# thunlp/OpenMatch

Measured on NVIDIA H100. Metric: queries/sec top-1000 over 8.8M x 768 corpus, higher is better.
Workload: dtype f16

## Files before the change

openmatch_b200/csrc/ptx.cuh:

```cuda
#pragma once
#include <cuda_runtime.h>
#include <cuda_bf16.h>
#include <stdint.h>

#ifndef OM_WAIT_TIMEOUT_CYCLES
#define OM_WAIT_TIMEOUT_CYCLES (1000000000ll)
#endif

namespace om {

static __device__ unsigned int om_dev_fault;

__device__ __forceinline__ uint32_t smem_u32(const void* p) {
  return static_cast<uint32_t>(__cvta_generic_to_shared(p));
}

__device__ __forceinline__ void mbar_init(uint64_t* bar, uint32_t count) {
  asm volatile("mbarrier.init.shared::cta.b64 [%0], %1;" ::"r"(smem_u32(bar)), "r"(count) : "memory");
}
__device__ __forceinline__ void fence_barrier_init() {
  asm volatile("fence.mbarrier_init.release.cluster;" ::: "memory");
}
__device__ __forceinline__ void fence_proxy_async_smem() {
  asm volatile("fence.proxy.async.shared::cta;" ::: "memory");
}
__device__ __forceinline__ void fence_proxy_async_global() {
  asm volatile("fence.proxy.async.global;" ::: "memory");
}
__device__ __forceinline__ void mbar_arrive_expect_tx(uint64_t* bar, uint32_t bytes) {
  asm volatile("mbarrier.arrive.expect_tx.shared::cta.b64 _, [%0], %1;" ::"r"(smem_u32(bar)), "r"(bytes)
               : "memory");
}
__device__ __forceinline__ void mbar_arrive(uint64_t* bar) {
  asm volatile("mbarrier.arrive.shared::cta.b64 _, [%0];" ::"r"(smem_u32(bar)) : "memory");
}
__device__ __forceinline__ bool mbar_try_wait(uint64_t* bar, uint32_t parity) {
  uint32_t done;
  asm volatile(
      "{\n\t"
      ".reg .pred P;\n\t"
      "mbarrier.try_wait.parity.shared::cta.b64 P, [%1], %2;\n\t"
      "selp.u32 %0, 1, 0, P;\n\t"
      "}\n"
      : "=r"(done)
      : "r"(smem_u32(bar)), "r"(parity)
      : "memory");
  return done != 0;
}
static __device__ __noinline__ void mbar_wait_slow(uint64_t* bar, uint32_t parity, uint32_t site) {
  const long long t0 = clock64();
  uint32_t spins = 0;
  while (!mbar_try_wait(bar, parity)) {
    if ((++spins & 1023u) != 0) continue;
    if (*reinterpret_cast<volatile unsigned int*>(&om_dev_fault) != 0u) return;
    if (clock64() - t0 > OM_WAIT_TIMEOUT_CYCLES) {
      atomicCAS(&om_dev_fault, 0u, (site << 16) | (blockIdx.x & 0xffffu) | 0x80000000u);
      return;
    }
  }
}
__device__ __forceinline__ void mbar_wait(uint64_t* bar, uint32_t parity, uint32_t site) {
  if (mbar_try_wait(bar, parity)) return;
  if (mbar_try_wait(bar, parity)) return;
  mbar_wait_slow(bar, parity, site);
}
__device__ __forceinline__ void mbar_wait_warp(uint64_t* bar, uint32_t parity, uint32_t site) {
  if ((threadIdx.x & 31u) == 0) {
    if (!mbar_try_wait(bar, parity)) {
      const long long t0 = clock64();
      uint32_t spins = 0;
      while (!mbar_try_wait(bar, parity)) {
        __nanosleep(64);
        if ((++spins & 1023u) != 0) continue;
        if (*reinterpret_cast<volatile unsigned int*>(&om_dev_fault) != 0u) break;
        if (clock64() - t0 > OM_WAIT_TIMEOUT_CYCLES) {
          atomicCAS(&om_dev_fault, 0u, (site << 16) | (blockIdx.x & 0xffffu) | 0x80000000u);
          break;
        }
      }
    }
  }
  __syncwarp();
}
static inline unsigned int read_clear_dev_fault() {
  unsigned int v = 0, z = 0;
  if (cudaMemcpyFromSymbol(&v, om_dev_fault, sizeof(v)) != cudaSuccess) return 0xffffffffu;
  if (v) cudaMemcpyToSymbol(om_dev_fault, &z, sizeof(z));
  return v;
}

__device__ __forceinline__ void tma_prefetch_desc(const void* tmap) {
  asm volatile("prefetch.tensormap [%0];" ::"l"(reinterpret_cast<uint64_t>(tmap)) : "memory");
}
__device__ __forceinline__ void tma_load_2d(void* smem_dst, const void* tmap, uint64_t* bar, int32_t c0,
                                            int32_t c1) {
  asm volatile(
      "cp.async.bulk.tensor.2d.shared::cluster.global.tile.mbarrier::complete_tx::bytes"
      " [%0], [%1, {%3, %4}], [%2];"
      ::"r"(smem_u32(smem_dst)), "l"(reinterpret_cast<uint64_t>(tmap)), "r"(smem_u32(bar)), "r"(c0), "r"(c1)
      : "memory");
}
__device__ __forceinline__ void tma_prefetch_l2_2d(const void* tmap, int32_t c0, int32_t c1) {
  asm volatile("cp.async.bulk.prefetch.tensor.2d.L2.global.tile [%0, {%1, %2}];" ::"l"(reinterpret_cast<uint64_t>(tmap)),
               "r"(c0), "r"(c1)
               : "memory");
}
__device__ __forceinline__ void tma_store_2d(const void* tmap, const void* smem_src, int32_t c0, int32_t c1) {
  asm volatile("cp.async.bulk.tensor.2d.global.shared::cta.tile.bulk_group [%0, {%2, %3}], [%1];" ::"l"(
                   reinterpret_cast<uint64_t>(tmap)),
               "r"(smem_u32(smem_src)), "r"(c0), "r"(c1)
               : "memory");
}
__device__ __forceinline__ void bulk_commit_group() { asm volatile("cp.async.bulk.commit_group;" ::: "memory"); }
__device__ __forceinline__ void bulk_wait_group_read0() { asm volatile("cp.async.bulk.wait_group.read 0;" ::: "memory"); }
__device__ __forceinline__ void bulk_wait_group0() { asm volatile("cp.async.bulk.wait_group 0;" ::: "memory"); }

__device__ __forceinline__ void tma_load_2d_multicast(void* smem_dst, const void* tmap, uint64_t* bar, int32_t c0,
                                                      int32_t c1, uint16_t cta_mask) {
  asm volatile(
      "cp.async.bulk.tensor.2d.shared::cluster.global.tile.mbarrier::complete_tx::bytes.multicast::cluster"
      " [%0], [%1, {%3, %4}], [%2], %5;"
      ::"r"(smem_u32(smem_dst)), "l"(reinterpret_cast<uint64_t>(tmap)), "r"(smem_u32(bar)), "r"(c0), "r"(c1),
      "h"(cta_mask)
      : "memory");
}

__device__ __forceinline__ uint32_t cluster_ctarank() {
  uint32_t r;
  asm volatile("mov.u32 %0, %%cluster_ctarank;" : "=r"(r));
  return r;
}
__device__ __forceinline__ uint32_t cluster_id_x() {
  uint32_t r;
  asm volatile("mov.u32 %0, %%clusterid.x;" : "=r"(r));
  return r;
}
__device__ __forceinline__ uint32_t cluster_count_x() {
  uint32_t r;
  asm volatile("mov.u32 %0, %%nclusterid.x;" : "=r"(r));
  return r;
}
__device__ __forceinline__ void cluster_sync_all() {
  asm volatile("barrier.cluster.arrive.release.aligned;\n\tbarrier.cluster.wait.acquire.aligned;" ::: "memory");
}
__device__ __forceinline__ void mbar_arrive_remote(uint64_t* bar, uint32_t rank) {
  asm volatile(
      "{\n\t.reg .b32 ra;\n\t"
      "mapa.shared::cluster.u32 ra, %0, %1;\n\t"
      "mbarrier.arrive.shared::cluster.b64 _, [ra];\n\t}\n"
      ::"r"(smem_u32(bar)), "r"(rank)
      : "memory");
}

__device__ __forceinline__ void wgmma_fence() { asm volatile("wgmma.fence.sync.aligned;" ::: "memory"); }
__device__ __forceinline__ void wgmma_commit() { asm volatile("wgmma.commit_group.sync.aligned;" ::: "memory"); }
template <int N>
__device__ __forceinline__ void wgmma_wait() {
  asm volatile("wgmma.wait_group.sync.aligned %0;" ::"n"(N) : "memory");
}
template <int R>
__device__ __forceinline__ void wgmma_fence_regs(float (&d)[R]) {
#pragma unroll
  for (int i = 0; i < R; ++i) asm volatile("" : "+f"(d[i])::"memory");
}

__host__ __device__ constexpr uint64_t wgmma_desc_base(uint32_t lbo_bytes, uint32_t sbo_bytes) {
  return (static_cast<uint64_t>((lbo_bytes >> 4) & 0x3fffu) << 16) |
         (static_cast<uint64_t>((sbo_bytes >> 4) & 0x3fffu) << 32) | (1ull << 62);
}
__device__ __forceinline__ uint64_t wgmma_desc(uint32_t smem_addr, uint64_t base) {
  return base | static_cast<uint64_t>((smem_addr & 0x3ffffu) >> 4);
}
constexpr uint64_t kDescKMajorSW128 = wgmma_desc_base(16, 1024);

template <int TA, int TB>
__device__ __forceinline__ void wgmma_m64n128k16_bf16(float (&d)[64], uint64_t a_desc, uint64_t b_desc, uint32_t accumulate) {
  asm volatile(
      "{\n\t.reg .pred p;\n\tsetp.ne.b32 p, %66, 0;\n\t"
      "wgmma.mma_async.sync.aligned.m64n128k16.f32.bf16.bf16 {%0, %1, %2, %3, %4, %5, %6, %7, %8, %9, %10, %11, %12, %13, %14, %15, %16, %17, %18, %19, %20, %21, %22, %23, %24, %25, %26, %27, %28, %29, %30, %31, %32, %33, %34, %35, %36, %37, %38, %39, %40, %41, %42, %43, %44, %45, %46, %47, %48, %49, %50, %51, %52, %53, %54, %55, %56, %57, %58, %59, %60, %61, %62, %63}, %64, %65, p, 1, 1, %67, %68;\n\t}\n"
      : "+f"(d[0]), "+f"(d[1]), "+f"(d[2]), "+f"(d[3]), "+f"(d[4]), "+f"(d[5]), "+f"(d[6]), "+f"(d[7]), "+f"(d[8]), "+f"(d[9]), "+f"(d[10]), "+f"(d[11]), "+f"(d[12]), "+f"(d[13]), "+f"(d[14]), "+f"(d[15]), "+f"(d[16]), "+f"(d[17]), "+f"(d[18]), "+f"(d[19]), "+f"(d[20]), "+f"(d[21]), "+f"(d[22]), "+f"(d[23]), "+f"(d[24]), "+f"(d[25]), "+f"(d[26]), "+f"(d[27]), "+f"(d[28]), "+f"(d[29]), "+f"(d[30]), "+f"(d[31]), "+f"(d[32]), "+f"(d[33]), "+f"(d[34]), "+f"(d[35]), "+f"(d[36]), "+f"(d[37]), "+f"(d[38]), "+f"(d[39]), "+f"(d[40]), "+f"(d[41]), "+f"(d[42]), "+f"(d[43]), "+f"(d[44]), "+f"(d[45]), "+f"(d[46]), "+f"(d[47]), "+f"(d[48]), "+f"(d[49]), "+f"(d[50]), "+f"(d[51]), "+f"(d[52]), "+f"(d[53]), "+f"(d[54]), "+f"(d[55]), "+f"(d[56]), "+f"(d[57]), "+f"(d[58]), "+f"(d[59]), "+f"(d[60]), "+f"(d[61]), "+f"(d[62]), "+f"(d[63])
      : "l"(a_desc), "l"(b_desc), "r"(accumulate), "n"(TA), "n"(TB));
}
template <int TA, int TB>
__device__ __forceinline__ void wgmma_m64n128k16_f16(float (&d)[64], uint64_t a_desc, uint64_t b_desc, uint32_t accumulate) {
  asm volatile(
      "{\n\t.reg .pred p;\n\tsetp.ne.b32 p, %66, 0;\n\t"
      "wgmma.mma_async.sync.aligned.m64n128k16.f32.f16.f16 {%0, %1, %2, %3, %4, %5, %6, %7, %8, %9, %10, %11, %12, %13, %14, %15, %16, %17, %18, %19, %20, %21, %22, %23, %24, %25, %26, %27, %28, %29, %30, %31, %32, %33, %34, %35, %36, %37, %38, %39, %40, %41, %42, %43, %44, %45, %46, %47, %48, %49, %50, %51, %52, %53, %54, %55, %56, %57, %58, %59, %60, %61, %62, %63}, %64, %65, p, 1, 1, %67, %68;\n\t}\n"
      : "+f"(d[0]), "+f"(d[1]), "+f"(d[2]), "+f"(d[3]), "+f"(d[4]), "+f"(d[5]), "+f"(d[6]), "+f"(d[7]), "+f"(d[8]), "+f"(d[9]), "+f"(d[10]), "+f"(d[11]), "+f"(d[12]), "+f"(d[13]), "+f"(d[14]), "+f"(d[15]), "+f"(d[16]), "+f"(d[17]), "+f"(d[18]), "+f"(d[19]), "+f"(d[20]), "+f"(d[21]), "+f"(d[22]), "+f"(d[23]), "+f"(d[24]), "+f"(d[25]), "+f"(d[26]), "+f"(d[27]), "+f"(d[28]), "+f"(d[29]), "+f"(d[30]), "+f"(d[31]), "+f"(d[32]), "+f"(d[33]), "+f"(d[34]), "+f"(d[35]), "+f"(d[36]), "+f"(d[37]), "+f"(d[38]), "+f"(d[39]), "+f"(d[40]), "+f"(d[41]), "+f"(d[42]), "+f"(d[43]), "+f"(d[44]), "+f"(d[45]), "+f"(d[46]), "+f"(d[47]), "+f"(d[48]), "+f"(d[49]), "+f"(d[50]), "+f"(d[51]), "+f"(d[52]), "+f"(d[53]), "+f"(d[54]), "+f"(d[55]), "+f"(d[56]), "+f"(d[57]), "+f"(d[58]), "+f"(d[59]), "+f"(d[60]), "+f"(d[61]), "+f"(d[62]), "+f"(d[63])
      : "l"(a_desc), "l"(b_desc), "r"(accumulate), "n"(TA), "n"(TB));
}
template <int TA, int TB>
__device__ __forceinline__ void wgmma_m64n256k16_f16(float (&d)[128], uint64_t a_desc, uint64_t b_desc, uint32_t accumulate) {
  asm volatile(
      "{\n\t.reg .pred p;\n\tsetp.ne.b32 p, %130, 0;\n\t"
      "wgmma.mma_async.sync.aligned.m64n256k16.f32.f16.f16 {%0, %1, %2, %3, %4, %5, %6, %7, %8, %9, %10, %11, %12, %13, %14, %15, %16, %17, %18, %19, %20, %21, %22, %23, %24, %25, %26, %27, %28, %29, %30, %31, %32, %33, %34, %35, %36, %37, %38, %39, %40, %41, %42, %43, %44, %45, %46, %47, %48, %49, %50, %51, %52, %53, %54, %55, %56, %57, %58, %59, %60, %61, %62, %63, %64, %65, %66, %67, %68, %69, %70, %71, %72, %73, %74, %75, %76, %77, %78, %79, %80, %81, %82, %83, %84, %85, %86, %87, %88, %89, %90, %91, %92, %93, %94, %95, %96, %97, %98, %99, %100, %101, %102, %103, %104, %105, %106, %107, %108, %109, %110, %111, %112, %113, %114, %115, %116, %117, %118, %119, %120, %121, %122, %123, %124, %125, %126, %127}, %128, %129, p, 1, 1, %131, %132;\n\t}\n"
      : "+f"(d[0]), "+f"(d[1]), "+f"(d[2]), "+f"(d[3]), "+f"(d[4]), "+f"(d[5]), "+f"(d[6]), "+f"(d[7]), "+f"(d[8]), "+f"(d[9]), "+f"(d[10]), "+f"(d[11]), "+f"(d[12]), "+f"(d[13]), "+f"(d[14]), "+f"(d[15]), "+f"(d[16]), "+f"(d[17]), "+f"(d[18]), "+f"(d[19]), "+f"(d[20]), "+f"(d[21]), "+f"(d[22]), "+f"(d[23]), "+f"(d[24]), "+f"(d[25]), "+f"(d[26]), "+f"(d[27]), "+f"(d[28]), "+f"(d[29]), "+f"(d[30]), "+f"(d[31]), "+f"(d[32]), "+f"(d[33]), "+f"(d[34]), "+f"(d[35]), "+f"(d[36]), "+f"(d[37]), "+f"(d[38]), "+f"(d[39]), "+f"(d[40]), "+f"(d[41]), "+f"(d[42]), "+f"(d[43]), "+f"(d[44]), "+f"(d[45]), "+f"(d[46]), "+f"(d[47]), "+f"(d[48]), "+f"(d[49]), "+f"(d[50]), "+f"(d[51]), "+f"(d[52]), "+f"(d[53]), "+f"(d[54]), "+f"(d[55]), "+f"(d[56]), "+f"(d[57]), "+f"(d[58]), "+f"(d[59]), "+f"(d[60]), "+f"(d[61]), "+f"(d[62]), "+f"(d[63]), "+f"(d[64]), "+f"(d[65]), "+f"(d[66]), "+f"(d[67]), "+f"(d[68]), "+f"(d[69]), "+f"(d[70]), "+f"(d[71]), "+f"(d[72]), "+f"(d[73]), "+f"(d[74]), "+f"(d[75]), "+f"(d[76]), "+f"(d[77]), "+f"(d[78]), "+f"(d[79]), "+f"(d[80]), "+f"(d[81]), "+f"(d[82]), "+f"(d[83]), "+f"(d[84]), "+f"(d[85]), "+f"(d[86]), "+f"(d[87]), "+f"(d[88]), "+f"(d[89]), "+f"(d[90]), "+f"(d[91]), "+f"(d[92]), "+f"(d[93]), "+f"(d[94]), "+f"(d[95]), "+f"(d[96]), "+f"(d[97]), "+f"(d[98]), "+f"(d[99]), "+f"(d[100]), "+f"(d[101]), "+f"(d[102]), "+f"(d[103]), "+f"(d[104]), "+f"(d[105]), "+f"(d[106]), "+f"(d[107]), "+f"(d[108]), "+f"(d[109]), "+f"(d[110]), "+f"(d[111]), "+f"(d[112]), "+f"(d[113]), "+f"(d[114]), "+f"(d[115]), "+f"(d[116]), "+f"(d[117]), "+f"(d[118]), "+f"(d[119]), "+f"(d[120]), "+f"(d[121]), "+f"(d[122]), "+f"(d[123]), "+f"(d[124]), "+f"(d[125]), "+f"(d[126]), "+f"(d[127])
      : "l"(a_desc), "l"(b_desc), "r"(accumulate), "n"(TA), "n"(TB));
}

template <int N>
__device__ __forceinline__ void setmaxnreg_dec() {
  asm volatile("setmaxnreg.dec.sync.aligned.u32 %0;" ::"n"(N));
}
template <int N>
__device__ __forceinline__ void setmaxnreg_inc() {
  asm volatile("setmaxnreg.inc.sync.aligned.u32 %0;" ::"n"(N));
}
__device__ __forceinline__ void wgmma_m64n64k16_bf16_rs(float (&d)[32], const uint32_t (&a)[4], uint64_t b_desc, uint32_t accumulate) {
  asm volatile(
      "{\n\t.reg .pred p;\n\tsetp.ne.b32 p, %37, 0;\n\t"
      "wgmma.mma_async.sync.aligned.m64n64k16.f32.bf16.bf16 {%0, %1, %2, %3, %4, %5, %6, %7, %8, %9, %10, %11, %12, %13, %14, %15, %16, %17, %18, %19, %20, %21, %22, %23, %24, %25, %26, %27, %28, %29, %30, %31}, {%32, %33, %34, %35}, %36, p, 1, 1, 0;\n\t}\n"
      : "+f"(d[0]), "+f"(d[1]), "+f"(d[2]), "+f"(d[3]), "+f"(d[4]), "+f"(d[5]), "+f"(d[6]), "+f"(d[7]), "+f"(d[8]), "+f"(d[9]), "+f"(d[10]), "+f"(d[11]), "+f"(d[12]), "+f"(d[13]), "+f"(d[14]), "+f"(d[15]), "+f"(d[16]), "+f"(d[17]), "+f"(d[18]), "+f"(d[19]), "+f"(d[20]), "+f"(d[21]), "+f"(d[22]), "+f"(d[23]), "+f"(d[24]), "+f"(d[25]), "+f"(d[26]), "+f"(d[27]), "+f"(d[28]), "+f"(d[29]), "+f"(d[30]), "+f"(d[31])
      : "r"(a[0]), "r"(a[1]), "r"(a[2]), "r"(a[3]), "l"(b_desc), "r"(accumulate));
}

__device__ __forceinline__ uint32_t pack_bf16x2(float lo, float hi) {
  __nv_bfloat162 v = __floats2bfloat162_rn(lo, hi);
  return *reinterpret_cast<uint32_t*>(&v);
}
__device__ __forceinline__ float2 fma2(float2 a, float2 b, float2 c) { return make_float2(fmaf(a.x, b.x, c.x), fmaf(a.y, b.y, c.y)); }
__device__ __forceinline__ float2 mul2(float2 a, float2 b) { return make_float2(__fmul_rn(a.x, b.x), __fmul_rn(a.y, b.y)); }
__device__ __forceinline__ float2 splat2(float x) { return make_float2(x, x); }

__device__ __forceinline__ void named_bar_sync(uint32_t id, uint32_t nthreads) {
  asm volatile("bar.sync %0, %1;" ::"r"(id), "r"(nthreads) : "memory");
}

}
```

openmatch_b200/csrc/scan_gemm.cuh:

```cuda
#pragma once
#include <cuda_fp16.h>

#include "scan_epilogue.cuh"

namespace om {

constexpr int kScanBlockN = 256;
constexpr int kScanStages = 3;
constexpr int kScanABytes = kBlockM * kBlockK * 2;
constexpr int kScanBBytes = kScanBlockN * kBlockK * 2;
constexpr int kScanStageBytes = kScanABytes + kScanBBytes;
constexpr int kScanConsumers = 256;
constexpr int kScanStash = 4;
constexpr int kScanStashOffset = kScanStages * kScanStageBytes;
constexpr int kScanStashBytes = 2 * 2 * kScanStash * kScanConsumers * 8;
constexpr int kScanBarOffset = kScanStashOffset + kScanStashBytes;
constexpr int kScanSmemBytes = kScanBarOffset + 2 * kScanStages * 8 + 1024;
static_assert(kScanSmemBytes <= 232448, "scan ring + stash exceed the 227 KB of shared memory an H100 block may use");

template <int H>
__device__ __forceinline__ float scan_pick(const float (&acc)[128], int i) {
  float a[32], b[16], c[8], d[4], e[2];
#pragma unroll
  for (int j = 0; j < 32; ++j) a[j] = (i & 1) ? acc[4 * j + 2 * H + 1] : acc[4 * j + 2 * H];
#pragma unroll
  for (int j = 0; j < 16; ++j) b[j] = (i & 2) ? a[2 * j + 1] : a[2 * j];
#pragma unroll
  for (int j = 0; j < 8; ++j) c[j] = (i & 4) ? b[2 * j + 1] : b[2 * j];
#pragma unroll
  for (int j = 0; j < 4; ++j) d[j] = (i & 8) ? c[2 * j + 1] : c[2 * j];
#pragma unroll
  for (int j = 0; j < 2; ++j) e[j] = (i & 16) ? d[2 * j + 1] : d[2 * j];
  return (i & 32) ? e[1] : e[0];
}

template <int H>
__device__ __forceinline__ int scan_filter_row(const float (&acc)[128], float t, int row, int lim, int q4, int col0,
                                               unsigned long long* stash, unsigned long long* cand, int* count,
                                               int* overflow, int C, uint32_t row_base) {
  float mx = acc[2 * H];
#pragma unroll
  for (int j = 0; j < 32; ++j) mx = fmaxf(mx, fmaxf(acc[4 * j + 2 * H], acc[4 * j + 2 * H + 1]));
  if (!(mx > t)) return 0;
  uint32_t lo = 0, hi = 0;
#pragma unroll
  for (int i = 0; i < 32; ++i) {
    lo |= (acc[4 * (i >> 1) + 2 * H + (i & 1)] > t ? 1u : 0u) << i;
    hi |= (acc[4 * (16 + (i >> 1)) + 2 * H + (i & 1)] > t ? 1u : 0u) << i;
  }
  unsigned long long mask = (static_cast<unsigned long long>(hi) << 32) | lo;
  if (lim < kScanBlockN) {
#pragma unroll 1
    for (int i = 0; i < 64; ++i)
      if (8 * (i >> 1) + 2 * q4 + (i & 1) >= lim) mask &= ~(1ull << i);
  }
  const int n = __popcll(mask);
  int pos = 0;
  if (n > kScanStash) {
    pos = atomicAdd(count + row, n - kScanStash);
    if (pos + (n - kScanStash) > C) *overflow = 1;
  }
  unsigned long long* mine = cand + static_cast<size_t>(row) * C;
  int idx = 0;
#pragma unroll 1
  while (mask) {
    const int i = __ffsll(static_cast<long long>(mask)) - 1;
    mask &= mask - 1;
    const unsigned long long key =
        make_key(scan_pick<H>(acc, i), row_base + static_cast<uint32_t>(col0 + 8 * (i >> 1) + 2 * q4 + (i & 1)));
    if (idx < kScanStash)
      stash[idx * kScanConsumers] = key;
    else if (pos + idx - kScanStash < C)
      mine[pos + idx - kScanStash] = key;
    ++idx;
  }
  return n < kScanStash ? n : kScanStash;
}

template <int CQ, int CX>
struct ScanCluster {
  static_assert((CQ == 2 || CQ == 4) && (CX == 1 || CX == 2), "scan cluster shapes: CQ in {2, 4}, CX in {1, 2}");
  static constexpr int kSize = CQ * CX;
  static constexpr int kShare = CQ + CX - 1;
  static constexpr int kQRows = kBlockM / CX;
  static constexpr int kXRows = kScanBlockN / CQ;
  static constexpr int kEmptyArrivals = kShare * (kScanConsumers / 32);
  __device__ static uint32_t peer_rank(uint32_t rank, int j) {
    const uint32_t a = rank % CQ, b = rank / CQ;
    if (j < CQ - 1) {
      const uint32_t o = static_cast<uint32_t>(j);
      return (o < a ? o : o + 1) + CQ * b;
    }
    const uint32_t o = static_cast<uint32_t>(j - (CQ - 1));
    return a + CQ * (o < b ? o : o + 1);
  }
  __device__ static uint16_t q_mask(uint32_t rank) {
    uint32_t m = 0;
#pragma unroll
    for (int b = 0; b < CX; ++b) m |= 1u << (rank % CQ + CQ * b);
    return static_cast<uint16_t>(m);
  }
  __device__ static uint16_t x_mask(uint32_t rank) {
    return static_cast<uint16_t>(((1u << CQ) - 1u) << (CQ * (rank / CQ)));
  }
};

template <int CQ, int CX>
__global__ void __launch_bounds__(kGemmProducerThreads + kScanConsumers, 1)
scan_wide_kernel(const __grid_constant__ CUtensorMap tmQ, const __grid_constant__ CUtensorMap tmX, int K,
                 const float* __restrict__ thr, unsigned long long* cand, int* count, int* overflow, int nq, int n_cols,
                 int C, uint32_t row_base) {
  using Cl = ScanCluster<CQ, CX>;
  extern __shared__ uint8_t smem_raw[];
  uint8_t* smem = reinterpret_cast<uint8_t*>((reinterpret_cast<uintptr_t>(smem_raw) + 1023) & ~uintptr_t(1023));
  unsigned long long* stash = reinterpret_cast<unsigned long long*>(smem + kScanStashOffset);
  uint64_t* full_bar = reinterpret_cast<uint64_t*>(smem + kScanBarOffset);
  uint64_t* empty_bar = full_bar + kScanStages;
  const uint32_t rank = cluster_ctarank();
  const int qa = static_cast<int>(rank % CQ), xb = static_cast<int>(rank / CQ);
  const int warp = __shfl_sync(0xffffffffu, static_cast<int>(threadIdx.x >> 5), 0);
  const int lane = static_cast<int>(threadIdx.x & 31);

  if (warp == 0 && lane == 0) {
    tma_prefetch_desc(&tmQ);
    tma_prefetch_desc(&tmX);
  }
  if (warp == 1 && lane == 0) {
    ring_init(full_bar, empty_bar, kScanStages, Cl::kEmptyArrivals);
    fence_barrier_init();
  }
  cluster_sync_all();

  const int qgroups = (nq + CQ * kBlockM - 1) / (CQ * kBlockM);
  const int num_tiles = qgroups * ((n_cols + CX * kScanBlockN - 1) / (CX * kScanBlockN));
  const int num_k = (K + kBlockK - 1) / kBlockK;

  if (warp < 4) {
    setmaxnreg_dec<40>();
    if (warp == 0 && lane == 0) {
      const uint16_t qmask = Cl::q_mask(rank), xmask = Cl::x_mask(rank);
      Ring<kScanStages> ring;
      for (int tile = static_cast<int>(cluster_id_x()); tile < num_tiles; tile += static_cast<int>(cluster_count_x())) {
        const int m_blk = (tile % qgroups) * CQ + qa;
        const int n_blk = (tile / qgroups) * CX + xb;
        for (int kb = 0; kb < num_k; ++kb) {
          uint64_t* bar = ring_acquire_tx(full_bar, empty_bar, ring, kScanStageBytes, 30);
          uint8_t* sa = smem + ring.stage * kScanStageBytes;
          if constexpr (CX == 1)
            tma_load_2d(sa, &tmQ, bar, kb * kBlockK, m_blk * kBlockM);
          else
            tma_load_2d_multicast(sa + xb * (Cl::kQRows * kBlockK * 2), &tmQ, bar, kb * kBlockK,
                                  m_blk * kBlockM + xb * Cl::kQRows, qmask);
          tma_load_2d_multicast(sa + kScanABytes + qa * (Cl::kXRows * kBlockK * 2), &tmX, bar, kb * kBlockK,
                                n_blk * kScanBlockN + qa * Cl::kXRows, xmask);
          ring.advance();
        }
      }
    }
  } else {
    setmaxnreg_inc<232>();
    const int et = static_cast<int>(threadIdx.x) - kGemmProducerThreads;
    const int wg = et >> 7;
    const int q4 = lane & 3;
    const int frow = 64 * wg + 16 * (warp & 3) + (lane >> 2);
    Ring<kScanStages> ring;
    int buf = 0;
    int p_n0 = 0, p_n1 = 0, p_excl0 = 0, p_excl1 = 0, p_pos0 = 0, p_pos1 = 0, p_row = 0, p_buf = 0;
    auto drain = [&]() {
      if (!__any_sync(0xffffffffu, (p_n0 | p_n1) != 0)) return;
      const int b0 = __shfl_sync(0xffffffffu, p_pos0, lane & ~3) + p_excl0;
      const int b1 = __shfl_sync(0xffffffffu, p_pos1, lane & ~3) + p_excl1;
      const unsigned long long* s = stash + p_buf * (2 * kScanStash * kScanConsumers) + et;
      unsigned long long* m0 = cand + static_cast<size_t>(p_row) * C;
      unsigned long long* m1 = cand + static_cast<size_t>(p_row + 8) * C;
      for (int j = 0; j < p_n0; ++j)
        if (b0 + j < C) m0[b0 + j] = s[j * kScanConsumers];
      for (int j = 0; j < p_n1; ++j)
        if (b1 + j < C) m1[b1 + j] = s[(kScanStash + j) * kScanConsumers];
      if ((p_n0 > 0 && b0 + p_n0 > C) || (p_n1 > 0 && b1 + p_n1 > C)) *overflow = 1;
      p_n0 = p_n1 = 0;
    };

    uint32_t peers[Cl::kShare - 1];
#pragma unroll
    for (int j = 0; j < Cl::kShare - 1; ++j) peers[j] = Cl::peer_rank(rank, j);
    auto release = [&](uint32_t s) {
      if (lane == 0) {
        mbar_arrive(&empty_bar[s]);
#pragma unroll
        for (int j = 0; j < Cl::kShare - 1; ++j) mbar_arrive_remote(&empty_bar[s], peers[j]);
      }
    };

    for (int tile = static_cast<int>(cluster_id_x()); tile < num_tiles; tile += static_cast<int>(cluster_count_x())) {
      const int m_blk = (tile % qgroups) * CQ + qa;
      const int n_blk = (tile / qgroups) * CX + xb;
      const int row0 = m_blk * kBlockM + frow, row1 = row0 + 8;
      const float inf = __int_as_float(0x7f800000);
      const float t0 = row0 < nq ? thr[row0] : inf, t1 = row1 < nq ? thr[row1] : inf;

      float acc[128];
#pragma unroll
      for (int i = 0; i < 128; ++i) acc[i] = 0.f;
      ring_consume(
          full_bar, ring, 0, num_k, 31,
          [&](uint32_t stage, uint32_t accumulate) {
            const uint32_t a_addr = smem_u32(smem + stage * kScanStageBytes) + wg * (64 * 128);
            const uint32_t b_addr = smem_u32(smem + stage * kScanStageBytes + kScanABytes);
#pragma unroll
            for (int k = 0; k < kBlockK / kWgmmaK; ++k)
              wgmma_m64n256k16_f16<0, 0>(acc, wgmma_desc(a_addr + k * 32, kDescKMajorSW128),
                                         wgmma_desc(b_addr + k * 32, kDescKMajorSW128), (accumulate | k) != 0 ? 1u : 0u);
          },
          release);
      wgmma_fence_regs(acc);

      drain();
      const int col0 = n_blk * kScanBlockN;
      const int lim = n_cols - col0;
      unsigned long long* sb = stash + buf * (2 * kScanStash * kScanConsumers) + et;
      const int k0 = scan_filter_row<0>(acc, t0, row0, lim, q4, col0, sb, cand, count, overflow, C, row_base);
      const int k1 = scan_filter_row<1>(acc, t1, row1, lim, q4, col0, sb + kScanStash * kScanConsumers, cand, count,
                                        overflow, C, row_base);
      if (__any_sync(0xffffffffu, (k0 | k1) != 0)) {
        int x0 = k0, x1 = k1;
        int y0 = __shfl_up_sync(0xffffffffu, x0, 1, 4), y1 = __shfl_up_sync(0xffffffffu, x1, 1, 4);
        if (q4 >= 1) x0 += y0, x1 += y1;
        y0 = __shfl_up_sync(0xffffffffu, x0, 2, 4), y1 = __shfl_up_sync(0xffffffffu, x1, 2, 4);
        if (q4 >= 2) x0 += y0, x1 += y1;
        const int n0 = __shfl_sync(0xffffffffu, x0, lane | 3), n1 = __shfl_sync(0xffffffffu, x1, lane | 3);
        if (q4 == 0) {
          if (n0 > 0) p_pos0 = atomicAdd(count + row0, n0);
          if (n1 > 0) p_pos1 = atomicAdd(count + row1, n1);
        }
        p_n0 = k0;
        p_n1 = k1;
        p_excl0 = x0 - k0;
        p_excl1 = x1 - k1;
        p_row = row0;
        p_buf = buf;
        buf ^= 1;
      }
    }
    drain();
  }

  __syncthreads();
  cluster_sync_all();
}

template <int CQ, int CX>
static inline cudaError_t scan_wide_max_clusters(int num_sms, int* out) {
  static int max_clusters = -1;
  if (max_clusters < 0) {
    constexpr int kSize = ScanCluster<CQ, CX>::kSize;
    cudaError_t e =
        cudaFuncSetAttribute(scan_wide_kernel<CQ, CX>, cudaFuncAttributeMaxDynamicSharedMemorySize, kScanSmemBytes);
    if (e != cudaSuccess) return e;
    cudaLaunchConfig_t cfg = {};
    cfg.gridDim = dim3(kSize * (num_sms / kSize));
    cfg.blockDim = dim3(kGemmProducerThreads + kScanConsumers);
    cfg.dynamicSmemBytes = kScanSmemBytes;
    cudaLaunchAttribute attr[1];
    attr[0].id = cudaLaunchAttributeClusterDimension;
    attr[0].val.clusterDim = {static_cast<unsigned>(kSize), 1, 1};
    cfg.attrs = attr;
    cfg.numAttrs = 1;
    int n = 0;
    e = cudaOccupancyMaxActiveClusters(&n, scan_wide_kernel<CQ, CX>, &cfg);
    if (e != cudaSuccess) return e;
    max_clusters = n < num_sms / kSize ? n : num_sms / kSize;
  }
  *out = max_clusters;
  return cudaSuccess;
}

template <int CQ, int CX>
static inline cudaError_t launch_scan_wide(const __half* Q, int64_t ldq, const __half* X, int64_t ldx, int nq, int n_cols,
                                           int K, const float* thr, unsigned long long* cand, int* count, int* overflow,
                                           int C, uint32_t row_base, int num_sms, cudaStream_t stream) {
  using Cl = ScanCluster<CQ, CX>;
  CUtensorMap tmQ, tmX;
  if (make_tmap_bf16_2d(&tmQ, Q, (uint64_t)K, (uint64_t)nq, (uint64_t)ldq * 2, kBlockK, Cl::kQRows) != 0)
    return cudaErrorInvalidValue;
  if (make_tmap_bf16_2d(&tmX, X, (uint64_t)K, (uint64_t)n_cols, (uint64_t)ldx * 2, kBlockK, Cl::kXRows) != 0)
    return cudaErrorInvalidValue;
  int max_clusters = 0;
  cudaError_t e = scan_wide_max_clusters<CQ, CX>(num_sms, &max_clusters);
  if (e != cudaSuccess) return e;
  if (max_clusters < 1) return cudaErrorNotSupported;
  cudaLaunchConfig_t cfg = {};
  cfg.blockDim = dim3(kGemmProducerThreads + kScanConsumers);
  cfg.dynamicSmemBytes = kScanSmemBytes;
  cfg.stream = stream;
  cudaLaunchAttribute attr[1];
  attr[0].id = cudaLaunchAttributeClusterDimension;
  attr[0].val.clusterDim = {static_cast<unsigned>(Cl::kSize), 1, 1};
  cfg.attrs = attr;
  cfg.numAttrs = 1;
  const int qgroups = (nq + CQ * kBlockM - 1) / (CQ * kBlockM);
  const int64_t num_tiles = static_cast<int64_t>(qgroups) * ((n_cols + CX * kScanBlockN - 1) / (CX * kScanBlockN));
  const int clusters = num_tiles < max_clusters ? static_cast<int>(num_tiles) : max_clusters;
  cfg.gridDim = dim3(Cl::kSize * clusters);
  return cudaLaunchKernelEx(&cfg, scan_wide_kernel<CQ, CX>, tmQ, tmX, K, thr, cand, count, overflow, nq, n_cols, C,
                            row_base);
}

static inline cudaError_t launch_scan_cluster(int cq, int cx, const __half* Q, int64_t ldq, const __half* X, int64_t ldx,
                                              int nq, int n_cols, int K, const float* thr, unsigned long long* cand,
                                              int* count, int* overflow, int C, uint32_t row_base, int num_sms,
                                              cudaStream_t stream) {
  if (nq <= 0 || n_cols <= 0 || K <= 0) return cudaSuccess;
  if (cq == 2 && cx == 1)
    return launch_scan_wide<2, 1>(Q, ldq, X, ldx, nq, n_cols, K, thr, cand, count, overflow, C, row_base, num_sms, stream);
  if (cq == 4 && cx == 1)
    return launch_scan_wide<4, 1>(Q, ldq, X, ldx, nq, n_cols, K, thr, cand, count, overflow, C, row_base, num_sms, stream);
  if (cq == 2 && cx == 2)
    return launch_scan_wide<2, 2>(Q, ldq, X, ldx, nq, n_cols, K, thr, cand, count, overflow, C, row_base, num_sms, stream);
  if (cq == 4 && cx == 2)
    return launch_scan_wide<4, 2>(Q, ldq, X, ldx, nq, n_cols, K, thr, cand, count, overflow, C, row_base, num_sms, stream);
  return cudaErrorInvalidValue;
}

static inline cudaError_t scan_cluster_capacity(int cq, int cx, int num_sms, int* out) {
  *out = -1;
  if (cq == 2 && cx == 1) return scan_wide_max_clusters<2, 1>(num_sms, out);
  if (cq == 4 && cx == 1) return scan_wide_max_clusters<4, 1>(num_sms, out);
  if (cq == 2 && cx == 2) return scan_wide_max_clusters<2, 2>(num_sms, out);
  if (cq == 4 && cx == 2) return scan_wide_max_clusters<4, 2>(num_sms, out);
  return cudaSuccess;
}

}
```

Before: 38290.

## Pipeline wgmma k-blocks with wait<1>, skip empty query tiles, drop accumulator zeroing

```diff
diff --git a/openmatch_b200/csrc/ptx.cuh b/openmatch_b200/csrc/ptx.cuh
--- a/openmatch_b200/csrc/ptx.cuh
+++ b/openmatch_b200/csrc/ptx.cuh
@@ -198,6 +198,14 @@
       : "l"(a_desc), "l"(b_desc), "r"(accumulate), "n"(TA), "n"(TB));
 }
 
+__device__ __forceinline__ void wgmma_m64n256k16_f16_first(float (&d)[128], uint64_t a_desc, uint64_t b_desc) {
+  asm volatile(
+      "{\n\t.reg .pred p;\n\tsetp.ne.b32 p, %130, 0;\n\t"
+      "wgmma.mma_async.sync.aligned.m64n256k16.f32.f16.f16 {%0, %1, %2, %3, %4, %5, %6, %7, %8, %9, %10, %11, %12, %13, %14, %15, %16, %17, %18, %19, %20, %21, %22, %23, %24, %25, %26, %27, %28, %29, %30, %31, %32, %33, %34, %35, %36, %37, %38, %39, %40, %41, %42, %43, %44, %45, %46, %47, %48, %49, %50, %51, %52, %53, %54, %55, %56, %57, %58, %59, %60, %61, %62, %63, %64, %65, %66, %67, %68, %69, %70, %71, %72, %73, %74, %75, %76, %77, %78, %79, %80, %81, %82, %83, %84, %85, %86, %87, %88, %89, %90, %91, %92, %93, %94, %95, %96, %97, %98, %99, %100, %101, %102, %103, %104, %105, %106, %107, %108, %109, %110, %111, %112, %113, %114, %115, %116, %117, %118, %119, %120, %121, %122, %123, %124, %125, %126, %127}, %128, %129, p, 1, 1, 0, 0;\n\t}\n"
+      : "=f"(d[0]), "=f"(d[1]), "=f"(d[2]), "=f"(d[3]), "=f"(d[4]), "=f"(d[5]), "=f"(d[6]), "=f"(d[7]), "=f"(d[8]), "=f"(d[9]), "=f"(d[10]), "=f"(d[11]), "=f"(d[12]), "=f"(d[13]), "=f"(d[14]), "=f"(d[15]), "=f"(d[16]), "=f"(d[17]), "=f"(d[18]), "=f"(d[19]), "=f"(d[20]), "=f"(d[21]), "=f"(d[22]), "=f"(d[23]), "=f"(d[24]), "=f"(d[25]), "=f"(d[26]), "=f"(d[27]), "=f"(d[28]), "=f"(d[29]), "=f"(d[30]), "=f"(d[31]), "=f"(d[32]), "=f"(d[33]), "=f"(d[34]), "=f"(d[35]), "=f"(d[36]), "=f"(d[37]), "=f"(d[38]), "=f"(d[39]), "=f"(d[40]), "=f"(d[41]), "=f"(d[42]), "=f"(d[43]), "=f"(d[44]), "=f"(d[45]), "=f"(d[46]), "=f"(d[47]), "=f"(d[48]), "=f"(d[49]), "=f"(d[50]), "=f"(d[51]), "=f"(d[52]), "=f"(d[53]), "=f"(d[54]), "=f"(d[55]), "=f"(d[56]), "=f"(d[57]), "=f"(d[58]), "=f"(d[59]), "=f"(d[60]), "=f"(d[61]), "=f"(d[62]), "=f"(d[63]), "=f"(d[64]), "=f"(d[65]), "=f"(d[66]), "=f"(d[67]), "=f"(d[68]), "=f"(d[69]), "=f"(d[70]), "=f"(d[71]), "=f"(d[72]), "=f"(d[73]), "=f"(d[74]), "=f"(d[75]), "=f"(d[76]), "=f"(d[77]), "=f"(d[78]), "=f"(d[79]), "=f"(d[80]), "=f"(d[81]), "=f"(d[82]), "=f"(d[83]), "=f"(d[84]), "=f"(d[85]), "=f"(d[86]), "=f"(d[87]), "=f"(d[88]), "=f"(d[89]), "=f"(d[90]), "=f"(d[91]), "=f"(d[92]), "=f"(d[93]), "=f"(d[94]), "=f"(d[95]), "=f"(d[96]), "=f"(d[97]), "=f"(d[98]), "=f"(d[99]), "=f"(d[100]), "=f"(d[101]), "=f"(d[102]), "=f"(d[103]), "=f"(d[104]), "=f"(d[105]), "=f"(d[106]), "=f"(d[107]), "=f"(d[108]), "=f"(d[109]), "=f"(d[110]), "=f"(d[111]), "=f"(d[112]), "=f"(d[113]), "=f"(d[114]), "=f"(d[115]), "=f"(d[116]), "=f"(d[117]), "=f"(d[118]), "=f"(d[119]), "=f"(d[120]), "=f"(d[121]), "=f"(d[122]), "=f"(d[123]), "=f"(d[124]), "=f"(d[125]), "=f"(d[126]), "=f"(d[127])
+      : "l"(a_desc), "l"(b_desc), "r"(0u));
+}
+
 template <int N>
 __device__ __forceinline__ void setmaxnreg_dec() {
   asm volatile("setmaxnreg.dec.sync.aligned.u32 %0;" ::"n"(N));
diff --git a/openmatch_b200/csrc/scan_gemm.cuh b/openmatch_b200/csrc/scan_gemm.cuh
--- a/openmatch_b200/csrc/scan_gemm.cuh
+++ b/openmatch_b200/csrc/scan_gemm.cuh
@@ -1,5 +1,7 @@
 #pragma once
 #include <cuda_fp16.h>
+
+#include <type_traits>
 
 #include "scan_epilogue.cuh"
 
@@ -195,24 +197,45 @@
     for (int tile = static_cast<int>(cluster_id_x()); tile < num_tiles; tile += static_cast<int>(cluster_count_x())) {
       const int m_blk = (tile % qgroups) * CQ + qa;
       const int n_blk = (tile / qgroups) * CX + xb;
+      if (m_blk * kBlockM >= nq) {
+        for (int kb = 0; kb < num_k; ++kb) {
+          mbar_wait_warp(&full_bar[ring.stage], ring.phase, 31);
+          release(ring.stage);
+          ring.advance();
+        }
+        continue;
+      }
       const int row0 = m_blk * kBlockM + frow, row1 = row0 + 8;
       const float inf = __int_as_float(0x7f800000);
       const float t0 = row0 < nq ? thr[row0] : inf, t1 = row1 < nq ? thr[row1] : inf;
 
       float acc[128];
-#pragma unroll
-      for (int i = 0; i < 128; ++i) acc[i] = 0.f;
-      ring_consume(
-          full_bar, ring, 0, num_k, 31,
-          [&](uint32_t stage, uint32_t accumulate) {
-            const uint32_t a_addr = smem_u32(smem + stage * kScanStageBytes) + wg * (64 * 128);
-            const uint32_t b_addr = smem_u32(smem + stage * kScanStageBytes + kScanABytes);
-#pragma unroll
-            for (int k = 0; k < kBlockK / kWgmmaK; ++k)
-              wgmma_m64n256k16_f16<0, 0>(acc, wgmma_desc(a_addr + k * 32, kDescKMajorSW128),
-                                         wgmma_desc(b_addr + k * 32, kDescKMajorSW128), (accumulate | k) != 0 ? 1u : 0u);
-          },
-          release);
+      uint32_t prev_stage = 0;
+      auto block = [&](auto first) {
+        mbar_wait_warp(&full_bar[ring.stage], ring.phase, 31);
+        const uint32_t a_addr = smem_u32(smem + ring.stage * kScanStageBytes) + wg * (64 * 128);
+        const uint32_t b_addr = smem_u32(smem + ring.stage * kScanStageBytes + kScanABytes);
+        wgmma_fence();
+#pragma unroll
+        for (int k = 0; k < kBlockK / kWgmmaK; ++k) {
+          const uint64_t da = wgmma_desc(a_addr + k * 32, kDescKMajorSW128), db = wgmma_desc(b_addr + k * 32, kDescKMajorSW128);
+          if (decltype(first)::value && k == 0)
+            wgmma_m64n256k16_f16_first(acc, da, db);
+          else
+            wgmma_m64n256k16_f16<0, 0>(acc, da, db, 1u);
+        }
+        wgmma_commit();
+        if constexpr (!decltype(first)::value) {
+          wgmma_wait<1>();
+          release(prev_stage);
+        }
+        prev_stage = ring.stage;
+        ring.advance();
+      };
+      block(std::true_type{});
+      for (int kb = 1; kb < num_k; ++kb) block(std::false_type{});
+      wgmma_wait<0>();
+      release(prev_stage);
       wgmma_fence_regs(acc);
 
       drain();
```

After: 38540, median of 6. About the same (+0.7%).
